# fims9000/SYNT_ISIC

Hardware: AMD Instinct MI355X
Metric: images/sec at 3x64x64 T=1000 (DDPM reverse-diffusion sampling) (higher is better)
Workload: dtype f32

## Files before the change

### synt_isic_amd/csrc/attention.hip

```cpp
#include <cstdlib>
#include <type_traits>

#include "common.h"

namespace sisic {

typedef float f32x16 __attribute__((ext_vector_type(16)));
typedef float f32x2 __attribute__((ext_vector_type(2)));
typedef short att_bf16x8 __attribute__((ext_vector_type(8)));
typedef unsigned att_u4 __attribute__((ext_vector_type(4)));
typedef unsigned att_u2 __attribute__((ext_vector_type(2)));

__device__ __forceinline__ void att_split2(float a, float b, unsigned& hi, unsigned& mid, unsigned& lo) {
    const unsigned ha = __float_as_uint(a) & 0xffff0000u, hb = __float_as_uint(b) & 0xffff0000u;
    const float ra = a - __uint_as_float(ha), rb = b - __uint_as_float(hb);
    const unsigned ma = __float_as_uint(ra) & 0xffff0000u, mb = __float_as_uint(rb) & 0xffff0000u;
    const float la = ra - __uint_as_float(ma), lb = rb - __uint_as_float(mb);
    hi = __builtin_amdgcn_perm(hb, ha, 0x07060302u);
    mid = __builtin_amdgcn_perm(mb, ma, 0x07060302u);
    lo = __builtin_amdgcn_perm(__float_as_uint(lb), __float_as_uint(la), 0x07060302u);
}

constexpr int ATT_D = 8;
constexpr int ATT_KB = 256;
constexpr int ATT_KT = ATT_KB / 32;
constexpr int ATT_WAVES = 4;

template <int QB>
__global__ void __launch_bounds__(64 * ATT_WAVES)
attention_kernel(const float* __restrict__ qkv, float* __restrict__ out, int C, int N, int heads, int q_blocks,
                 float scale) {
    __shared__ __attribute__((aligned(16))) unsigned Kh[2 * ATT_KB * 4];
    __shared__ __attribute__((aligned(16))) unsigned Kl[2 * ATT_KB * 2];
    __shared__ __attribute__((aligned(16))) float Vs[ATT_D * ATT_KB];

    int blk = blockIdx.x;
    const int qb = blk % q_blocks;
    blk /= q_blocks;
    const int head = blk % heads;
    const int b = blk / heads;

    const int tid = threadIdx.x, lane = tid & 63, wave = tid >> 6;
    const int half = lane >> 5, l31 = lane & 31;
    const int q0 = qb * (32 * QB * ATT_WAVES) + wave * (32 * QB);
    const bool wave_active = q0 < N;

    const float* Qp = qkv + ((size_t)b * 3 * C + (size_t)head * ATT_D) * N;
    const float* Kp = Qp + (size_t)C * N;
    const float* Vp = Kp + (size_t)C * N;

    att_u4 b_hm[QB], b_mh[QB], b_lh[QB];
#pragma unroll
    for (int j = 0; j < QB; ++j) {
        const int q = q0 + 32 * j + l31;
        float qv[4];
#pragma unroll
        for (int k = 0; k < 4; ++k) qv[k] = (q < N) ? Qp[(size_t)(4 * half + k) * N + q] * scale : 0.0f;
        unsigned h0, m0, l0, h1, m1, l1;
        att_split2(qv[0], qv[1], h0, m0, l0);
        att_split2(qv[2], qv[3], h1, m1, l1);
        b_hm[j] = att_u4{h0, h1, m0, m1};
        b_mh[j] = att_u4{m0, m1, h0, h1};
        b_lh[j] = att_u4{l0, l1, h0, h1};
    }

    float m_run[QB], l_part[QB];
    f32x2 o2[QB][ATT_D / 2];
#pragma unroll
    for (int j = 0; j < QB; ++j) {
        m_run[j] = -INFINITY; l_part[j] = 0.0f;
#pragma unroll
        for (int d = 0; d < ATT_D / 2; ++d) o2[j][d] = f32x2{0.0f, 0.0f};
    }

    auto tile = [&](const int kt, const int nk, auto masked) {
        constexpr bool MASKED = decltype(masked)::value;
        f32x16 S[QB];
        {
            const int key = half * ATT_KB + kt * 32 + l31;
            const att_u4 a_hm = *reinterpret_cast<const att_u4*>(&Kh[key * 4]);
            const att_u2 a_l = *reinterpret_cast<const att_u2*>(&Kl[key * 2]);
            const att_u4 a_hl = {a_hm.x, a_hm.y, a_l.x, a_l.y};
#pragma unroll
            for (int j = 0; j < QB; ++j) {
#pragma unroll
                for (int r = 0; r < 16; ++r) S[j][r] = 0.0f;
                S[j] = __builtin_amdgcn_mfma_f32_32x32x16_bf16(__builtin_bit_cast(att_bf16x8, a_hm), __builtin_bit_cast(att_bf16x8, b_hm[j]), S[j], 0, 0, 0);
                S[j] = __builtin_amdgcn_mfma_f32_32x32x16_bf16(__builtin_bit_cast(att_bf16x8, a_hm), __builtin_bit_cast(att_bf16x8, b_mh[j]), S[j], 0, 0, 0);
                S[j] = __builtin_amdgcn_mfma_f32_32x32x16_bf16(__builtin_bit_cast(att_bf16x8, a_hl), __builtin_bit_cast(att_bf16x8, b_lh[j]), S[j], 0, 0, 0);
            }
        }
        float m_new[QB];
#pragma unroll
        for (int j = 0; j < QB; ++j) {
            float tmax = -INFINITY;
#pragma unroll
            for (int r = 0; r < 16; ++r) {
                if (MASKED) {
                    const int key = kt * 32 + (r & 3) + 8 * (r >> 2) + 4 * half;
                    S[j][r] = (key < nk) ? S[j][r] : -INFINITY;
                }
                tmax = fmaxf(tmax, S[j][r]);
            }
            {
                const auto sw = __builtin_amdgcn_permlane32_swap(__float_as_uint(tmax), __float_as_uint(tmax), false, false);
                tmax = fmaxf(__uint_as_float(sw[0]), __uint_as_float(sw[1]));
            }
            m_new[j] = fmaxf(m_run[j], tmax);
            const float alpha = __builtin_amdgcn_exp2f(m_run[j] - m_new[j]);
            asm("s_nop 1\n\tv_mul_f32 %0, %1, %2" : "=v"(l_part[j]) : "v"(l_part[j]), "v"(alpha));
            const f32x2 a2 = f32x2{alpha, alpha};
#pragma unroll
            for (int d = 0; d < ATT_D / 2; ++d) asm("s_nop 1\n\tv_pk_mul_f32 %0, %1, %2" : "=v"(o2[j][d]) : "v"(o2[j][d]), "v"(a2));
            m_run[j] = m_new[j];
        }
#pragma unroll
        for (int rq = 0; rq < 4; ++rq) {
            float pv[QB][4];
#pragma unroll
            for (int j = 0; j < QB; ++j) {
                const f32x2 mm = f32x2{m_new[j], m_new[j]};
                const f32x2 d0 = f32x2{S[j][4 * rq], S[j][4 * rq + 1]} - mm, d1 = f32x2{S[j][4 * rq + 2], S[j][4 * rq + 3]} - mm;
                pv[j][0] = __builtin_amdgcn_exp2f(d0.x); pv[j][1] = __builtin_amdgcn_exp2f(d0.y);
                pv[j][2] = __builtin_amdgcn_exp2f(d1.x); pv[j][3] = __builtin_amdgcn_exp2f(d1.y);
                l_part[j] += (pv[j][0] + pv[j][1]) + (pv[j][2] + pv[j][3]);
            }
            const int koff = kt * 32 + 8 * rq + 4 * half;
#pragma unroll
            for (int i = 0; i < 4; ++i) {
                const float4 va = *reinterpret_cast<const float4*>(&Vs[(koff + i) * ATT_D]);
                const float4 vb = *reinterpret_cast<const float4*>(&Vs[(koff + i) * ATT_D + 4]);
#pragma unroll
                for (int j = 0; j < QB; ++j) {
                    const f32x2 p2 = f32x2{pv[j][i], pv[j][i]};
                    o2[j][0] += p2 * f32x2{va.x, va.y};
                    o2[j][1] += p2 * f32x2{va.z, va.w};
                    o2[j][2] += p2 * f32x2{vb.x, vb.y};
                    o2[j][3] += p2 * f32x2{vb.z, vb.w};
                }
            }
        }
    };

    for (int kb0 = 0; kb0 < N; kb0 += ATT_KB) {
        __syncthreads();
        for (int idx = tid; idx < 2 * ATT_KB; idx += 64 * ATT_WAVES) {
            const int g = idx / ATT_KB, k = idx % ATT_KB;
            const int key = kb0 + k;
            float kv[4];
#pragma unroll
            for (int d = 0; d < 4; ++d) kv[d] = key < N ? Kp[(size_t)(4 * g + d) * N + key] : 0.0f;
            unsigned h0, m0, l0, h1, m1, l1;
            att_split2(kv[0], kv[1], h0, m0, l0);
            att_split2(kv[2], kv[3], h1, m1, l1);
            *reinterpret_cast<att_u4*>(&Kh[idx * 4]) = att_u4{h0, h1, m0, m1};
            *reinterpret_cast<att_u2*>(&Kl[idx * 2]) = att_u2{l0, l1};
        }
        for (int k = tid; k < ATT_KB; k += 64 * ATT_WAVES) {
            const int key = kb0 + k;
            float v[ATT_D];
#pragma unroll
            for (int d = 0; d < ATT_D; ++d) v[d] = key < N ? Vp[(size_t)d * N + key] : 0.0f;
            *reinterpret_cast<float4*>(&Vs[k * ATT_D]) = make_float4(v[0], v[1], v[2], v[3]);
            *reinterpret_cast<float4*>(&Vs[k * ATT_D + 4]) = make_float4(v[4], v[5], v[6], v[7]);
        }
        __syncthreads();
        if (!wave_active) continue;
        const int nk = min(ATT_KB, N - kb0);
#pragma unroll 1
        for (int kt = 0; kt * 32 < nk; ++kt) {
            if (kt * 32 + 32 <= nk) tile(kt, nk, std::false_type{});
            else tile(kt, nk, std::true_type{});
        }
    }

    if (wave_active) {
#pragma unroll
        for (int j = 0; j < QB; ++j) {
            const int q = q0 + 32 * j + l31;
            float o[ATT_D];
#pragma unroll
            for (int d = 0; d < ATT_D / 2; ++d) { o[2 * d] = o2[j][d].x; o[2 * d + 1] = o2[j][d].y; }
            const float l_tot = l_part[j] + __shfl_xor(l_part[j], 32, 64);
            const float inv = 1.0f / l_tot;
            float res[ATT_D];
#pragma unroll
            for (int d = 0; d < ATT_D; ++d) res[d] = (o[d] + __shfl_xor(o[d], 32, 64)) * inv;
            if (q < N) {
                float* Op = out + ((size_t)b * C + (size_t)head * ATT_D) * N + q;
#pragma unroll
                for (int dd = 0; dd < 4; ++dd) {
                    const int hm = -half;
                    const float v = __int_as_float((__float_as_int(res[dd]) & ~hm) | (__float_as_int(res[4 + dd]) & hm));
                    Op[(size_t)(4 * half + dd) * N] = v;
                }
            }
        }
    }
}

int launch_attention(sisic_ctx* ctx, const float* qkv, float* out, int B, int C, int N, int head_dim, hipStream_t s) {
    SISIC_REQUIRE(qkv && out, "attention: null tensor");
    if (head_dim == 32 || head_dim == 64) return launch_attention_wide(ctx, qkv, out, B, C, N, head_dim, s);
    SISIC_REQUIRE(head_dim == ATT_D, "attention: head_dim %d unsupported (8, 32 and 64 have kernels)", head_dim);
    SISIC_REQUIRE(B > 0 && N > 0 && C > 0 && C % head_dim == 0, "attention: bad shape B=%d C=%d N=%d", B, C, N);
    const int heads = C / head_dim;
    static const int qb_env = [] { const char* e = std::getenv("SISIC_ATT_QB"); return e ? std::atoi(e) : 0; }();
    const int cus = ctx->num_cus > 0 ? ctx->num_cus : 256;
    const int qb = qb_env == 1 || qb_env == 2 ? qb_env : ((int64_t)B * heads * cdiv(N, 64 * ATT_WAVES) >= 4 * (int64_t)cus ? 2 : 1);
    const int q_blocks = cdiv(N, 32 * qb * ATT_WAVES);
    const int64_t grid = (int64_t)B * heads * q_blocks;
    SISIC_REQUIRE(grid < (int64_t(1) << 31), "attention: grid too large");
    ProfileScope prof(ctx, s, PK_ATTN, 16.0 * B * C * N, 4.0 * B * C * double(N) * N);
    const float scale = 1.4426950408889634f / sqrtf((float)head_dim);
    if (qb == 2)
        hipLaunchKernelGGL(attention_kernel<2>, dim3((unsigned)grid), dim3(64 * ATT_WAVES), 0, s, qkv, out, C, N, heads, q_blocks, scale);
    else
        hipLaunchKernelGGL(attention_kernel<1>, dim3((unsigned)grid), dim3(64 * ATT_WAVES), 0, s, qkv, out, C, N, heads, q_blocks, scale);
    SISIC_HIP(hipGetLastError());
    return SISIC_OK;
}

}
```

### synt_isic_amd/csrc/conv_pointwise_bf3.hip

```cpp
#include <cstdlib>
#include <type_traits>

#include "conv_plan.h"
#include "gn_finalize.h"

namespace sisic {

typedef float pwb_f32x16 __attribute__((ext_vector_type(16)));
typedef short pwb_bf16x8 __attribute__((ext_vector_type(8)));
typedef unsigned pwb_u4 __attribute__((ext_vector_type(4)));
typedef unsigned pwb_u2 __attribute__((ext_vector_type(2)));
typedef float pwb_f2 __attribute__((ext_vector_type(2)));
typedef float pwb_f4 __attribute__((ext_vector_type(4)));

struct PwbParams {
    const float* in0;
    const float* in1;
    int c0, c1, B, HW;
    const float* wb;
    int n_co64;
    const float* bias;
    int Cout;
    const float* gn_scale;
    const float* gn_shift;
// ... 246 lines not shown
            if (p.bias) add[r] += p.bias[col];
            if (p.chan_bias) add[r] += p.chan_bias[(size_t)b * p.chan_bias_stride + col];
            res[r] = pwb_f2{0.0f, 0.0f};
            if (p.residual) {
                if constexpr (NB == 2) res[r] = __builtin_bit_cast(pwb_f2, __builtin_amdgcn_raw_buffer_load_b64(rsr, o_voff, 4u * (unsigned)(cs * HW), 0));
                else res[r].x = __builtin_bit_cast(float, __builtin_amdgcn_raw_buffer_load_b32(rsr, o_voff, 4u * (unsigned)(cs * HW), 0));
            }
        }
#pragma unroll
        for (int r = 0; r < 16; ++r) {
            const int cs = co0 + 32 * x + 8 * (r >> 2) + (r & 3);
            float vv[2] = {0.0f, 0.0f};
#pragma unroll
            for (int nb = 0; nb < NB; ++nb) {
                vv[nb] = acc[x][nb][r] + add[r] + (nb ? res[r].y : res[r].x);
                if (p.relu) vv[nb] = fmaxf(vv[nb], 0.0f);
            }
            if constexpr (NB == 2) __builtin_amdgcn_raw_buffer_store_b64(pwb_u2{__float_as_uint(vv[0]), __float_as_uint(vv[1])}, rso, o_voff, 4u * (unsigned)(cs * HW), 0);
            else __builtin_amdgcn_raw_buffer_store_b32(__float_as_uint(vv[0]), rso, o_voff, 4u * (unsigned)(cs * HW), 0);
            if (p.stats) {
                const int co = cs + 4 * half;
                if constexpr (NB == 1) {
                    const float s1 = pwb_half_wave_sum(vv[0]);
                    const float d = vv[0] - s1 * (1.0f / 32.0f);
                    float dd;
                    asm volatile("v_mul_f32 %0, %1, %1" : "=v"(dd) : "v"(d));
                    const float q = pwb_half_wave_sum(dd);
                    if (l31 == 0)
                        reinterpret_cast<float4*>(p.stats)[((size_t)b * p.Cout + co) * slots + px_t] = make_float4(32.0f, s1, q, 0.0f);
                } else {
                    const float s1 = pwb_row16_sum(vv[0] + vv[1]);
                    const float mean = s1 * (1.0f / 32.0f);
                    const float d0 = vv[0] - mean, d1 = vv[1] - mean;
                    float q0, q1;
                    asm volatile("v_mul_f32 %0, %2, %2\n\tv_mul_f32 %1, %3, %3" : "=&v"(q0), "=&v"(q1) : "v"(d0), "v"(d1));
                    const float q = pwb_row16_sum(q0 + q1);
                    if ((l31 & 15) == 0)
                        reinterpret_cast<float4*>(p.stats)[((size_t)b * p.Cout + co) * slots + 2 * px_t + (l31 >> 4)] = make_float4(32.0f, s1, q, 0.0f);
                }
            }
        }
    }
}

#ifndef PWBK_VAR
#define PWBK_VAR 0
#endif
template <int PRO>
__global__ void __launch_bounds__(64 * PWB_WAVES, 4) conv_pwbk_kernel(const PwbParams p) {
    extern __shared__ __attribute__((aligned(16))) float smem[];
    int L = blockIdx.x;
    if constexpr (PRO == 0) {
        if (L < p.n_rider_wg) {
            gn_finalize_job(p.rider, L * GNF_WAVES + (int)(threadIdx.x >> 6), threadIdx.x & 63);
            return;
        }
        L -= p.n_rider_wg;
    }
    int item;
    {
        const int nwg = p.nwg;
        const int xcd = L & 7, slot = L >> 3, q = nwg >> 3, r = nwg & 7;
        item = (xcd < r ? xcd * (q + 1) : r * (q + 1) + (xcd - r) * q) + slot;
    }
    const int tid = threadIdx.x, lane = tid & 63;
    const int wave_u = __builtin_amdgcn_readfirstlane(tid >> 6);
    const int half = lane >> 5, l31 = lane & 31;
    int co_i = item % p.n_co_items;
    const int t = item / p.n_co_items;
    int px_t = t % p.n_px, b = t / p.n_px;
    asm volatile("" : "+s"(co_i), "+s"(px_t), "+s"(b));
    constexpr int CB = 2;
    const int px0 = 32 * px_t, co0 = 64 * co_i;
    const int Cin = p.c0 + p.c1, HW = p.HW;
    const int nl = p.nchunks / PWB_WAVES, cb = wave_u * nl;

    const __amdgpu_buffer_rsrc_t rs0 = __builtin_amdgcn_make_buffer_rsrc(const_cast<float*>(p.in0 + (size_t)b * p.c0 * HW), 0, -1, 0x00020000);
    const __amdgpu_buffer_rsrc_t rs1 = __builtin_amdgcn_make_buffer_rsrc(
        const_cast<float*>(p.in1 ? p.in1 + (size_t)b * p.c1 * HW : p.in0), 0, -1, 0x00020000);
    const __amdgpu_buffer_rsrc_t rsw = __builtin_amdgcn_make_buffer_rsrc(const_cast<float*>(p.wb), 0, -1, 0x00020000);
    const unsigned x_voff = 4u * (unsigned)((4 * half) * HW + px0 + l31);
    const unsigned a_lane16 = 16u * (unsigned)lane, a_lane8 = 8u * (unsigned)lane;

    float* const P_lds = smem;
    float* const gnL = smem + PWB_WAVES * 32 * 64 + wave_u * (2 * 8 * nl);
    if constexpr (PRO != 0) {
        for (int i = lane; i < 8 * nl; i += 64) {
            gnL[2 * i] = p.gn_scale[(size_t)b * Cin + 8 * cb + i];
            gnL[2 * i + 1] = p.gn_shift[(size_t)b * Cin + 8 * cb + i];
        }
        asm volatile("s_waitcnt lgkmcnt(0)" ::: "memory");
        __builtin_amdgcn_wave_barrier();
    }

    pwb_f32x16 acc[CB];
#pragma unroll
    for (int x = 0; x < CB; ++x)
#pragma unroll
        for (int r = 0; r < 16; ++r) acc[x][r] = 0.0f;
    struct XRegs { float x[4]; };
    auto load_x = [&](int c, XRegs& r) {
        const int cc0 = 8 * c;
        if (cc0 < p.c0) {
            const unsigned soff = 4u * (unsigned)(cc0 * HW);
#pragma unroll
            for (int k = 0; k < 4; ++k) r.x[k] = __builtin_bit_cast(float, __builtin_amdgcn_raw_buffer_load_b32(rs0, x_voff, soff + 4u * (unsigned)(k * HW), 0));
        } else {
            const unsigned soff = 4u * (unsigned)((cc0 - p.c0) * HW);
#pragma unroll
            for (int k = 0; k < 4; ++k) r.x[k] = __builtin_bit_cast(float, __builtin_amdgcn_raw_buffer_load_b32(rs1, x_voff, soff + 4u * (unsigned)(k * HW), 0));
        }
    };
    auto load_f = [&](int c, pwb_u4 (&fa)[CB], pwb_u2 (&fl)[CB]) {
        const unsigned s0 = 3072u * (unsigned)(c * p.n_co64 + co_i);
#pragma unroll
        for (int x = 0; x < CB; ++x) {
            fa[x] = __builtin_amdgcn_raw_buffer_load_b128(rsw, a_lane16, s0 + 1024u * (unsigned)x, 0);
#if (PWBK_VAR & 1) != 0
            fl[x] = pwb_u2{fa[x].z, fa[x].w};
#else
            fl[x] = __builtin_amdgcn_raw_buffer_load_b64(rsw, a_lane8, s0 + 2048u + 512u * (unsigned)x, 0);
#endif
#if (PWBK_VAR & 2) != 0
            fa[x] = pwb_u4{a_lane16 + (unsigned)c, a_lane8, s0, a_lane16 ^ s0};
            fl[x] = pwb_u2{fa[x].z, fa[x].w};
#endif
        }
    };
    struct Tup { pwb_u4 hm, mh, lh; };
    auto make = [&](int cl, const XRegs& r) {
        pwb_f4 g01 = {1.0f, 0.0f, 1.0f, 0.0f}, g23 = g01;
        if constexpr (PRO != 0) {
            const float* gp = gnL + 2 * (8 * cl + 4 * half);
            g01 = *reinterpret_cast<const pwb_f4*>(gp);
            g23 = *reinterpret_cast<const pwb_f4*>(gp + 4);
        }
        float v[4];
#pragma unroll
        for (int k = 0; k < 4; ++k) {
            float e = r.x[k];
            if constexpr (PRO != 0) {
                const float sc = k == 0 ? g01.x : (k == 1 ? g01.z : (k == 2 ? g23.x : g23.z));
                const float sh = k == 0 ? g01.y : (k == 1 ? g01.w : (k == 2 ? g23.y : g23.w));
                e = e * sc + sh;
                if constexpr (PRO == 2) e = pwb_silu(e);
            }
            v[k] = e;
        }
        unsigned hi[2], mid[2], lo[2];
#pragma unroll
        for (int q = 0; q < 2; ++q) {
            const float v0 = v[2 * q], v1 = v[2 * q + 1];
            const unsigned h0 = __float_as_uint(v0) & 0xffff0000u, h1 = __float_as_uint(v1) & 0xffff0000u;
            const float r0 = v0 - __uint_as_float(h0), r1 = v1 - __uint_as_float(h1);
            const unsigned m0 = __float_as_uint(r0) & 0xffff0000u, m1 = __float_as_uint(r1) & 0xffff0000u;
            const float l0 = r0 - __uint_as_float(m0), l1 = r1 - __uint_as_float(m1);
            hi[q] = __builtin_amdgcn_perm(h1, h0, 0x07060302u);
            mid[q] = __builtin_amdgcn_perm(m1, m0, 0x07060302u);
            lo[q] = __builtin_amdgcn_perm(__float_as_uint(l1), __float_as_uint(l0), 0x07060302u);
        }
        return Tup{pwb_u4{hi[0], hi[1], mid[0], mid[1]}, pwb_u4{mid[0], mid[1], hi[0], hi[1]}, pwb_u4{lo[0], lo[1], hi[0], hi[1]}};
    };
    auto mm = [&](const Tup& t, const pwb_u4 (&fa)[CB], const pwb_u2 (&fl)[CB]) {
#pragma unroll
        for (int x = 0; x < CB; ++x) {
            const pwb_u4 a_hl = {fa[x].x, fa[x].y, fl[x].x, fl[x].y};
            acc[x] = __builtin_amdgcn_mfma_f32_32x32x16_bf16(__builtin_bit_cast(pwb_bf16x8, fa[x]), __builtin_bit_cast(pwb_bf16x8, t.hm), acc[x], 0, 0, 0);
            acc[x] = __builtin_amdgcn_mfma_f32_32x32x16_bf16(__builtin_bit_cast(pwb_bf16x8, fa[x]), __builtin_bit_cast(pwb_bf16x8, t.mh), acc[x], 0, 0, 0);
            acc[x] = __builtin_amdgcn_mfma_f32_32x32x16_bf16(__builtin_bit_cast(pwb_bf16x8, a_hl), __builtin_bit_cast(pwb_bf16x8, t.lh), acc[x], 0, 0, 0);
        }
    };
    constexpr int XD = 4;
    XRegs xr[XD];
    pwb_u4 ua[CB], ub[CB];
    pwb_u2 ul[CB], um[CB];
#pragma unroll
    for (int i = 0; i < XD; ++i)
        if (i < nl) load_x(cb + i, xr[i]);
    load_f(cb, ua, ul);
    if (nl > 1) load_f(cb + 1, ub, um);
    for (int c = 0; c < nl; c += XD) {
#pragma unroll
        for (int i = 0; i < XD; ++i) {
            if (c + i < nl) {
                const Tup t = make(c + i, xr[i]);
                if (c + i + XD < nl) load_x(cb + c + i + XD, xr[i]);
                if ((i & 1) == 0) {
                    mm(t, ua, ul);
                    if (c + i + 2 < nl) load_f(cb + c + i + 2, ua, ul);
                } else {
                    mm(t, ub, um);
                    if (c + i + 2 < nl) load_f(cb + c + i + 2, ub, um);
                }
            }
        }
    }

#pragma unroll
    for (int x = 0; x < CB; ++x)
#pragma unroll
        for (int r = 0; r < 16; ++r) P_lds[((wave_u * 2 + x) * 16 + r) * 64 + lane] = acc[x][r];
    __syncthreads();
    const int x = wave_u >> 1, rb = 8 * (wave_u & 1);
    const __amdgpu_buffer_rsrc_t rso = __builtin_amdgcn_make_buffer_rsrc(p.out + (size_t)b * p.Cout * HW, 0, -1, 0x00020000);
    const __amdgpu_buffer_rsrc_t rsr = __builtin_amdgcn_make_buffer_rsrc(
        const_cast<float*>(p.residual ? p.residual + (size_t)b * p.Cout * HW : p.out), 0, -1, 0x00020000);
    const unsigned o_voff = 4u * (unsigned)((4 * half) * HW + px0 + l31);
    const int slots = HW / 32;
    float add[8], res[8];
#pragma unroll
    for (int rr = 0; rr < 8; ++rr) {
        const int r = rb + rr;
        const int cs = co0 + 32 * x + 8 * (r >> 2) + (r & 3);
        const int col = cs + 4 * half;
        add[rr] = 0.0f;
        if (p.bias) add[rr] += p.bias[col];
        if (p.chan_bias) add[rr] += p.chan_bias[(size_t)b * p.chan_bias_stride + col];
        res[rr] = 0.0f;
        if (p.residual) res[rr] = __builtin_bit_cast(float, __builtin_amdgcn_raw_buffer_load_b32(rsr, o_voff, 4u * (unsigned)(cs * HW), 0));
    }
#pragma unroll
    for (int rr = 0; rr < 8; ++rr) {
        const int r = rb + rr;
        const int cs = co0 + 32 * x + 8 * (r >> 2) + (r & 3);
        float part[PWB_WAVES];
#pragma unroll
        for (int k = 0; k < PWB_WAVES; ++k) part[k] = P_lds[((k * 2 + x) * 16 + r) * 64 + lane];
        float v = ((part[0] + part[1]) + part[2]) + part[3];
        v = v + add[rr] + res[rr];
        if (p.relu) v = fmaxf(v, 0.0f);
        __builtin_amdgcn_raw_buffer_store_b32(__float_as_uint(v), rso, o_voff, 4u * (unsigned)(cs * HW), 0);
        if (p.stats) {
            const int co = cs + 4 * half;
            const float s1 = pwb_half_wave_sum(v);
            const float d = v - s1 * (1.0f / 32.0f);
            float dd;
            asm volatile("v_mul_f32 %0, %1, %1" : "=v"(dd) : "v"(d));
            const float q = pwb_half_wave_sum(dd);
            if (l31 == 0)
                reinterpret_cast<float4*>(p.stats)[((size_t)b * p.Cout + co) * slots + px_t] = make_float4(32.0f, s1, q, 0.0f);
        }
    }
}

__device__ __forceinline__ void pwbs_load_chunk(const __amdgpu_buffer_rsrc_t rs0, const __amdgpu_buffer_rsrc_t rs1, const int c0, const int HW,
                                                const int c, const unsigned x_voff, pwb_f2 (&xr)[4]) {
    const int cc0 = 8 * c;
    if (cc0 < c0) {
        const unsigned soff = 4u * (unsigned)(cc0 * HW);
#pragma unroll
        for (int k = 0; k < 4; ++k) xr[k] = __builtin_bit_cast(pwb_f2, __builtin_amdgcn_raw_buffer_load_b64(rs0, x_voff, soff + 4u * (unsigned)(k * HW), 0));
    } else {
        const unsigned soff = 4u * (unsigned)((cc0 - c0) * HW);
#pragma unroll
        for (int k = 0; k < 4; ++k) xr[k] = __builtin_bit_cast(pwb_f2, __builtin_amdgcn_raw_buffer_load_b64(rs1, x_voff, soff + 4u * (unsigned)(k * HW), 0));
    }
}
template <int PRO>
__device__ __forceinline__ void pwbs_split_store(const pwb_f2 (&xr)[4], const float* gp, unsigned* const S_hm, unsigned* const S_lo, const int slot,
                                                 const int lane) {
    pwb_f4 g01 = {1.0f, 0.0f, 1.0f, 0.0f}, g23 = g01;
    if constexpr (PRO != 0) {
        g01 = *reinterpret_cast<const pwb_f4*>(gp);
        g23 = *reinterpret_cast<const pwb_f4*>(gp + 4);
    }
#pragma unroll
    for (int nb = 0; nb < 2; ++nb) {
        float v[4];
#pragma unroll
        for (int k = 0; k < 4; ++k) {
            float e = nb ? xr[k].y : xr[k].x;
            if constexpr (PRO != 0) {
                const float sc = k == 0 ? g01.x : (k == 1 ? g01.z : (k == 2 ? g23.x : g23.z));
                const float sh = k == 0 ? g01.y : (k == 1 ? g01.w : (k == 2 ? g23.y : g23.w));
                e = e * sc + sh;
                if constexpr (PRO == 2) e = pwb_silu(e);
            }
            v[k] = e;
        }
        unsigned hi[2], mid[2], lo[2];
#pragma unroll
        for (int q = 0; q < 2; ++q) {
            const float v0 = v[2 * q], v1 = v[2 * q + 1];
            const unsigned h0 = __float_as_uint(v0) & 0xffff0000u, h1 = __float_as_uint(v1) & 0xffff0000u;
            const float r0 = v0 - __uint_as_float(h0), r1 = v1 - __uint_as_float(h1);
            const unsigned m0 = __float_as_uint(r0) & 0xffff0000u, m1 = __float_as_uint(r1) & 0xffff0000u;
            const float l0 = r0 - __uint_as_float(m0), l1 = r1 - __uint_as_float(m1);
            hi[q] = __builtin_amdgcn_perm(h1, h0, 0x07060302u);
            mid[q] = __builtin_amdgcn_perm(m1, m0, 0x07060302u);
            lo[q] = __builtin_amdgcn_perm(__float_as_uint(l1), __float_as_uint(l0), 0x07060302u);
        }
        *reinterpret_cast<pwb_u4*>(S_hm + ((size_t)(slot * 2 + nb) * 64 + lane) * 4) = pwb_u4{hi[0], hi[1], mid[0], mid[1]};
        *reinterpret_cast<pwb_u2*>(S_lo + ((size_t)(slot * 2 + nb) * 64 + lane) * 2) = pwb_u2{lo[0], lo[1]};
    }
}
__device__ __forceinline__ void pwbs_read_b(const unsigned* const S_hm, const unsigned* const S_lo, const int slot, const int nb, const int lane,
                                            pwb_u4& hm, pwb_u4& mh, pwb_u4& lh) {
    hm = *reinterpret_cast<const pwb_u4*>(S_hm + ((size_t)(slot * 2 + nb) * 64 + lane) * 4);
    const pwb_u2 lo = *reinterpret_cast<const pwb_u2*>(S_lo + ((size_t)(slot * 2 + nb) * 64 + lane) * 2);
    mh = pwb_u4{hm.z, hm.w, hm.x, hm.y};
    lh = pwb_u4{lo.x, lo.y, hm.x, hm.y};
}

template <int PRO>
__global__ void __launch_bounds__(64 * PWBS_MAX_WAVES) conv_pwbs_kernel(const PwbParams p) {
    extern __shared__ __attribute__((aligned(16))) float smem[];
    int wg;
    {
        const int L = blockIdx.x, nwg = p.nwg;
        const int xcd = L & 7, slot = L >> 3, q = nwg >> 3, r = nwg & 7;
        wg = (xcd < r ? xcd * (q + 1) : r * (q + 1) + (xcd - r) * q) + slot;
    }
    const int tid = threadIdx.x, lane = tid & 63;
    const int wave_u = __builtin_amdgcn_readfirstlane(tid >> 6);
    const int nwaves = p.n_co_items;
    const int half = lane >> 5, l31 = lane & 31;
    int px_t = wg % p.n_px, b = wg / p.n_px;
    asm volatile("" : "+s"(px_t), "+s"(b));
    constexpr int CB = 2, NB = 2;
    const int co_i = wave_u;
    const int px0 = 64 * px_t, co0 = 64 * co_i;
    const int Cin = p.c0 + p.c1, HW = p.HW, n = p.nchunks;

    const __amdgpu_buffer_rsrc_t rs0 = __builtin_amdgcn_make_buffer_rsrc(const_cast<float*>(p.in0 + (size_t)b * p.c0 * HW), 0, -1, 0x00020000);
    const __amdgpu_buffer_rsrc_t rs1 = __builtin_amdgcn_make_buffer_rsrc(
        const_cast<float*>(p.in1 ? p.in1 + (size_t)b * p.c1 * HW : p.in0), 0, -1, 0x00020000);
    const __amdgpu_buffer_rsrc_t rsw = __builtin_amdgcn_make_buffer_rsrc(const_cast<float*>(p.wb), 0, -1, 0x00020000);
    const unsigned x_voff = 4u * (unsigned)((4 * half) * HW + px0 + NB * l31);
    const unsigned a_lane16 = 16u * (unsigned)lane, a_lane8 = 8u * (unsigned)lane;

    unsigned* const S_hm = reinterpret_cast<unsigned*>(smem);
    unsigned* const S_lo = S_hm + (size_t)n * NB * 64 * 4;
    float* const gnL = reinterpret_cast<float*>(S_lo + (size_t)n * NB * 64 * 2);
    if constexpr (PRO != 0) {
        for (int i = tid; i < Cin; i += 64 * nwaves) {
            gnL[2 * i] = p.gn_scale[(size_t)b * Cin + i];
            gnL[2 * i + 1] = p.gn_shift[(size_t)b * Cin + i];
        }
        __syncthreads();
    }
    for (int c = wave_u; c < n; c += nwaves) {
        pwb_f2 xr[4];
        pwbs_load_chunk(rs0, rs1, p.c0, HW, c, x_voff, xr);
        pwbs_split_store<PRO>(xr, gnL + 2 * (8 * c + 4 * half), S_hm, S_lo, c, lane);
    }
    __syncthreads();

    pwb_f32x16 acc[CB][NB];
#pragma unroll
    for (int x = 0; x < CB; ++x)
#pragma unroll
        for (int nb = 0; nb < NB; ++nb)
#pragma unroll
            for (int r = 0; r < 16; ++r) acc[x][nb][r] = 0.0f;
    pwb_u4 ua[CB], ub[CB];
    pwb_u2 ul[CB], um[CB];
    auto load_f = [&](int c, pwb_u4 (&fa)[CB], pwb_u2 (&fl)[CB]) {
        const unsigned s0 = 3072u * (unsigned)(c * p.n_co64 + co_i);
#pragma unroll
        for (int x = 0; x < CB; ++x) {
            fa[x] = __builtin_amdgcn_raw_buffer_load_b128(rsw, a_lane16, s0 + 1024u * (unsigned)x, 0);
            fl[x] = __builtin_amdgcn_raw_buffer_load_b64(rsw, a_lane8, s0 + 2048u + 512u * (unsigned)x, 0);
        }
    };
    auto chunk = [&](int c, const pwb_u4 (&fa)[CB], const pwb_u2 (&fl)[CB]) {
#pragma unroll
        for (int nb = 0; nb < NB; ++nb) {
            pwb_u4 hm, mh, lh;
            pwbs_read_b(S_hm, S_lo, c, nb, lane, hm, mh, lh);
#pragma unroll
            for (int x = 0; x < CB; ++x) {
                const pwb_u4 a_hl = {fa[x].x, fa[x].y, fl[x].x, fl[x].y};
                acc[x][nb] = __builtin_amdgcn_mfma_f32_32x32x16_bf16(__builtin_bit_cast(pwb_bf16x8, fa[x]), __builtin_bit_cast(pwb_bf16x8, hm), acc[x][nb], 0, 0, 0);
                acc[x][nb] = __builtin_amdgcn_mfma_f32_32x32x16_bf16(__builtin_bit_cast(pwb_bf16x8, fa[x]), __builtin_bit_cast(pwb_bf16x8, mh), acc[x][nb], 0, 0, 0);
                acc[x][nb] = __builtin_amdgcn_mfma_f32_32x32x16_bf16(__builtin_bit_cast(pwb_bf16x8, a_hl), __builtin_bit_cast(pwb_bf16x8, lh), acc[x][nb], 0, 0, 0);
            }
        }
    };
    load_f(0, ua, ul);
    if (n > 1) load_f(1, ub, um);
    {
        int c = 0;
        for (; c + 1 < n; c += 2) {
            chunk(c, ua, ul);
            if (c + 2 < n) load_f(c + 2, ua, ul);
            chunk(c + 1, ub, um);
            if (c + 3 < n) load_f(c + 3, ub, um);
        }
        if (c < n) chunk(c, ua, ul);
    }

    const __amdgpu_buffer_rsrc_t rso = __builtin_amdgcn_make_buffer_rsrc(p.out + (size_t)b * p.Cout * HW, 0, -1, 0x00020000);
    const __amdgpu_buffer_rsrc_t rsr = __builtin_amdgcn_make_buffer_rsrc(
        const_cast<float*>(p.residual ? p.residual + (size_t)b * p.Cout * HW : p.out), 0, -1, 0x00020000);
    const unsigned o_voff = 4u * (unsigned)((4 * half) * HW + px0 + NB * l31);
    const int slots = HW / 32;
#pragma unroll
    for (int x = 0; x < CB; ++x) {
        float add[16];
        pwb_f2 res[16];
#pragma unroll
        for (int r = 0; r < 16; ++r) {
            const int cs = co0 + 32 * x + 8 * (r >> 2) + (r & 3);
            const int col = cs + 4 * half;
            add[r] = 0.0f;
            if (p.bias) add[r] += p.bias[col];
            if (p.chan_bias) add[r] += p.chan_bias[(size_t)b * p.chan_bias_stride + col];
            res[r] = pwb_f2{0.0f, 0.0f};
            if (p.residual) res[r] = __builtin_bit_cast(pwb_f2, __builtin_amdgcn_raw_buffer_load_b64(rsr, o_voff, 4u * (unsigned)(cs * HW), 0));
        }
#pragma unroll
        for (int r = 0; r < 16; ++r) {
            const int cs = co0 + 32 * x + 8 * (r >> 2) + (r & 3);
            float vv[2];
#pragma unroll
            for (int nb = 0; nb < NB; ++nb) {
                vv[nb] = acc[x][nb][r] + add[r] + (nb ? res[r].y : res[r].x);
                if (p.relu) vv[nb] = fmaxf(vv[nb], 0.0f);
            }
            __builtin_amdgcn_raw_buffer_store_b64(pwb_u2{__float_as_uint(vv[0]), __float_as_uint(vv[1])}, rso, o_voff, 4u * (unsigned)(cs * HW), 0);
            if (p.stats) {
                const int co = cs + 4 * half;
                const float s1 = pwb_row16_sum(vv[0] + vv[1]);
                const float mean = s1 * (1.0f / 32.0f);
                const float d0 = vv[0] - mean, d1 = vv[1] - mean;
                float q0, q1;
                asm volatile("v_mul_f32 %0, %2, %2\n\tv_mul_f32 %1, %3, %3" : "=&v"(q0), "=&v"(q1) : "v"(d0), "v"(d1));
                const float q = pwb_row16_sum(q0 + q1);
                if ((l31 & 15) == 0)
                    reinterpret_cast<float4*>(p.stats)[((size_t)b * p.Cout + co) * slots + 2 * px_t + (l31 >> 4)] = make_float4(32.0f, s1, q, 0.0f);
            }
        }
    }
}

#ifndef PWBSK_VAR
#define PWBSK_VAR 0
#endif
__global__ void __launch_bounds__(64 * PWBSK_MAX_WAVES) conv_pwbsk_kernel(const PwbParams p) {
    extern __shared__ __attribute__((aligned(16))) float smem[];
    const int tid = threadIdx.x, lane = tid & 63;
    const int wave_u = __builtin_amdgcn_readfirstlane(tid >> 6);
    const int nwaves = PWB_WAVES * p.n_co_items;
    int L = blockIdx.x;
    if (L < p.n_rider_wg) {
        gn_finalize_job(p.rider, L * nwaves + wave_u, lane);
        return;
    }
    L -= p.n_rider_wg;
    int wg;
    {
        const int nwg = p.nwg;
        const int xcd = L & 7, slot = L >> 3, q = nwg >> 3, r = nwg & 7;
        wg = (xcd < r ? xcd * (q + 1) : r * (q + 1) + (xcd - r) * q) + slot;
    }
    const int half = lane >> 5, l31 = lane & 31;
    int px_t = wg % p.n_px, b = wg / p.n_px;
    asm volatile("" : "+s"(px_t), "+s"(b));
    constexpr int CB = 2, NB = 2;
    const int co_i = wave_u / PWB_WAVES, kq = wave_u % PWB_WAVES;
    const int px0 = 64 * px_t, co0 = 64 * co_i;
    const int HW = p.HW;
    const int nl = p.nchunks / PWB_WAVES, cb = kq * nl;
    const int cap = nl < PWBSK_CAP ? nl : PWBSK_CAP;

    const __amdgpu_buffer_rsrc_t rs0 = __builtin_amdgcn_make_buffer_rsrc(const_cast<float*>(p.in0 + (size_t)b * p.c0 * HW), 0, -1, 0x00020000);
    const __amdgpu_buffer_rsrc_t rs1 = __builtin_amdgcn_make_buffer_rsrc(
        const_cast<float*>(p.in1 ? p.in1 + (size_t)b * p.c1 * HW : p.in0), 0, -1, 0x00020000);
    const __amdgpu_buffer_rsrc_t rsw = __builtin_amdgcn_make_buffer_rsrc(const_cast<float*>(p.wb), 0, -1, 0x00020000);
    const unsigned x_voff = 4u * (unsigned)((4 * half) * HW + px0 + NB * l31);
    const unsigned a_lane16 = 16u * (unsigned)lane, a_lane8 = 8u * (unsigned)lane;

    unsigned* const S_hm = reinterpret_cast<unsigned*>(smem);
    unsigned* const S_lo = S_hm + (size_t)(PWB_WAVES * cap) * NB * 64 * 4;
    float* const P_lds = smem;

    pwb_f32x16 acc[CB][NB];
#pragma unroll
    for (int x = 0; x < CB; ++x)
#pragma unroll
        for (int nb = 0; nb < NB; ++nb)
#pragma unroll
            for (int r = 0; r < 16; ++r) acc[x][nb][r] = 0.0f;
    pwb_u4 ua[CB], ub[CB];
    pwb_u2 ul[CB], um[CB];
    auto load_f = [&](int c, pwb_u4 (&fa)[CB], pwb_u2 (&fl)[CB]) {
        const unsigned s0 = 3072u * (unsigned)(c * p.n_co64 + co_i);
#pragma unroll
        for (int x = 0; x < CB; ++x) {
#if (PWBSK_VAR & 8) != 0
            fa[x] = pwb_u4{a_lane16 + (unsigned)c, a_lane8, s0, a_lane16 ^ s0};
            fl[x] = pwb_u2{fa[x].z, fa[x].w};
#else
            fa[x] = __builtin_amdgcn_raw_buffer_load_b128(rsw, a_lane16, s0 + 1024u * (unsigned)x, 0);
            fl[x] = __builtin_amdgcn_raw_buffer_load_b64(rsw, a_lane8, s0 + 2048u + 512u * (unsigned)x, 0);
#endif
        }
    };
    auto chunk = [&](int slot, const pwb_u4 (&fa)[CB], const pwb_u2 (&fl)[CB]) {
#pragma unroll
        for (int nb = 0; nb < NB; ++nb) {
            pwb_u4 hm, mh, lh;
            pwbs_read_b(S_hm, S_lo, slot, nb, lane, hm, mh, lh);
#pragma unroll
            for (int x = 0; x < CB; ++x) {
                const pwb_u4 a_hl = {fa[x].x, fa[x].y, fl[x].x, fl[x].y};
                acc[x][nb] = __builtin_amdgcn_mfma_f32_32x32x16_bf16(__builtin_bit_cast(pwb_bf16x8, fa[x]), __builtin_bit_cast(pwb_bf16x8, hm), acc[x][nb], 0, 0, 0);
                acc[x][nb] = __builtin_amdgcn_mfma_f32_32x32x16_bf16(__builtin_bit_cast(pwb_bf16x8, fa[x]), __builtin_bit_cast(pwb_bf16x8, mh), acc[x][nb], 0, 0, 0);
                acc[x][nb] = __builtin_amdgcn_mfma_f32_32x32x16_bf16(__builtin_bit_cast(pwb_bf16x8, a_hl), __builtin_bit_cast(pwb_bf16x8, lh), acc[x][nb], 0, 0, 0);
            }
        }
    };
    load_f(cb, ua, ul);
    load_f(cb + 1, ub, um);
    for (int p0 = 0; p0 < nl; p0 += cap) {
        const int len = nl - p0 < cap ? nl - p0 : cap, nslots = PWB_WAVES * len;
        if (p0 != 0) __syncthreads();
#if (PWBSK_VAR & 1) == 0
        for (int t = wave_u; t < nslots; t += 2 * nwaves) {
            const int t1 = t + nwaves;
            pwb_f2 xa[4], xb[4];
            pwbs_load_chunk(rs0, rs1, p.c0, HW, (t / len) * nl + p0 + t % len, x_voff, xa);
            if (t1 < nslots) pwbs_load_chunk(rs0, rs1, p.c0, HW, (t1 / len) * nl + p0 + t1 % len, x_voff, xb);
            pwbs_split_store<0>(xa, nullptr, S_hm, S_lo, (t / len) * cap + t % len, lane);
            if (t1 < nslots) pwbs_split_store<0>(xb, nullptr, S_hm, S_lo, (t1 / len) * cap + t1 % len, lane);
        }
#endif
        __syncthreads();
#if (PWBSK_VAR & 2) == 0
        for (int j = 0; j < len; j += 2) {
            chunk(kq * cap + j, ua, ul);
            if (p0 + j + 2 < nl) load_f(cb + p0 + j + 2, ua, ul);
            chunk(kq * cap + j + 1, ub, um);
            if (p0 + j + 3 < nl) load_f(cb + p0 + j + 3, ub, um);
        }
#else
        acc[0][0][0] += __uint_as_float(ua[0].x ^ ub[1].y ^ ul[0].x ^ um[1].y) + __uint_as_float(S_hm[lane + 64 * kq]);
#endif
    }

    const __amdgpu_buffer_rsrc_t rso = __builtin_amdgcn_make_buffer_rsrc(p.out + (size_t)b * p.Cout * HW, 0, -1, 0x00020000);
    const __amdgpu_buffer_rsrc_t rsr = __builtin_amdgcn_make_buffer_rsrc(
        const_cast<float*>(p.residual ? p.residual + (size_t)b * p.Cout * HW : p.out), 0, -1, 0x00020000);
    const unsigned o_voff = 4u * (unsigned)((4 * half) * HW + px0 + NB * l31);
    const int slots = HW / 32;
#pragma unroll
    for (int x = 0; x < CB; ++x) {
#if (PWBSK_VAR & 4) == 0
        __syncthreads();
#pragma unroll
        for (int nb = 0; nb < NB; ++nb)
#pragma unroll
            for (int r = 0; r < 16; ++r) P_lds[((wave_u * NB + nb) * 16 + r) * 64 + lane] = acc[x][nb][r];
        __syncthreads();
#endif
        float add[4];
        pwb_f2 res[4];
#pragma unroll
        for (int rr = 0; rr < 4; ++rr) {
            const int cs = co0 + 32 * x + 8 * kq + rr;
            const int col = cs + 4 * half;
            add[rr] = 0.0f;
            if (p.bias) add[rr] += p.bias[col];
            if (p.chan_bias) add[rr] += p.chan_bias[(size_t)b * p.chan_bias_stride + col];
            res[rr] = pwb_f2{0.0f, 0.0f};
            if (p.residual) res[rr] = __builtin_bit_cast(pwb_f2, __builtin_amdgcn_raw_buffer_load_b64(rsr, o_voff, 4u * (unsigned)(cs * HW), 0));
        }
#pragma unroll
        for (int rr = 0; rr < 4; ++rr) {
            const int r = 4 * kq + rr;
            const int cs = co0 + 32 * x + 8 * kq + rr;
            float vv[NB];
#pragma unroll
            for (int nb = 0; nb < NB; ++nb) {
                float part[PWB_WAVES];
#if (PWBSK_VAR & 4) == 0
#pragma unroll
                for (int k = 0; k < PWB_WAVES; ++k) part[k] = P_lds[(((co_i * PWB_WAVES + k) * NB + nb) * 16 + r) * 64 + lane];
#else
#pragma unroll
                for (int k = 0; k < PWB_WAVES; ++k) part[k] = acc[x][nb][4 * k + rr];
#endif
                float v = ((part[0] + part[1]) + part[2]) + part[3];
                v = v + add[rr] + (nb ? res[rr].y : res[rr].x);
                vv[nb] = v;
            }
            __builtin_amdgcn_raw_buffer_store_b64(pwb_u2{__float_as_uint(vv[0]), __float_as_uint(vv[1])}, rso, o_voff, 4u * (unsigned)(cs * HW), 0);
            if (p.stats) {
                const int co = cs + 4 * half;
                const float s1 = pwb_row16_sum(vv[0] + vv[1]);
                const float mean = s1 * (1.0f / 32.0f);
                const float d0 = vv[0] - mean, d1 = vv[1] - mean;
                float q0, q1;
                asm volatile("v_mul_f32 %0, %2, %2\n\tv_mul_f32 %1, %3, %3" : "=&v"(q0), "=&v"(q1) : "v"(d0), "v"(d1));
                const float q = pwb_row16_sum(q0 + q1);
                if ((l31 & 15) == 0)
                    reinterpret_cast<float4*>(p.stats)[((size_t)b * p.Cout + co) * slots + 2 * px_t + (l31 >> 4)] = make_float4(32.0f, s1, q, 0.0f);
            }
        }
    }
}

static int launch_pwbsk(sisic_ctx* ctx, PwbParams& p, int Cin, hipStream_t s, const GnFinJob* rider) {
    p.n_co_items = p.Cout / 64;
    p.n_px = p.HW / 64;
    const int nwaves = PWB_WAVES * p.n_co_items;
    const int64_t nwg = (int64_t)p.B * p.n_px;
    p.n_rider_wg = rider ? cdiv(rider->n_jobs, nwaves) : 0;
    SISIC_REQUIRE(nwg > 0 && nwg + p.n_rider_wg < (int64_t(1) << 31), "conv2d(pointwise bf16x3, staged K-split): grid too large");
    p.nwg = (int)nwg;
    p.nitems = p.nwg * p.n_co_items;
    const size_t lds = pwbsk_lds_bytes(Cin, p.Cout);
    static std::atomic<uint64_t> opt{0};
    auto kern = conv_pwbsk_kernel;
    SISIC_TRY(ensure_dynamic_lds(ctx, reinterpret_cast<const void*>(kern), (int)PWBSK_MAX_LDS, opt));
    hipLaunchKernelGGL(kern, dim3(p.n_rider_wg + p.nwg), dim3(64 * nwaves), lds, s, p);
    SISIC_HIP(hipGetLastError());
    return SISIC_OK;
}

template <int PRO>
static int launch_pwbk(sisic_ctx* ctx, PwbParams& p, int Cin, hipStream_t s) {
    p.n_co_items = p.Cout / 64;
    p.n_px = p.HW / 32;
    const int64_t nitems = (int64_t)p.B * p.n_px * p.n_co_items;
    SISIC_REQUIRE(nitems > 0 && nitems < (int64_t(1) << 31), "conv2d(pointwise bf16x3, K-split): grid too large");
    p.nitems = (int)nitems;
    p.nwg = p.nitems;
    SISIC_REQUIRE((int64_t)p.nwg + p.n_rider_wg < (int64_t(1) << 31), "conv2d(pointwise bf16x3, K-split): grid too large");
    const size_t lds = sizeof(float) * (size_t)(PWB_WAVES * 32 * 64 + (PRO ? 2 * Cin : 0));
    static std::atomic<uint64_t> opt{0};
    auto kern = conv_pwbk_kernel<PRO>;
    SISIC_TRY(ensure_dynamic_lds(ctx, reinterpret_cast<const void*>(kern), (int)lds, opt));
    hipLaunchKernelGGL(kern, dim3(p.n_rider_wg + p.nwg), dim3(64 * PWB_WAVES), lds, s, p);
    SISIC_HIP(hipGetLastError());
    return SISIC_OK;
}

template <int PRO>
static int launch_pwbs(sisic_ctx* ctx, PwbParams& p, int Cin, hipStream_t s) {
    p.n_co_items = p.Cout / 64;
    p.n_px = p.HW / 64;
    const int64_t nwg = (int64_t)p.B * p.n_px;
    SISIC_REQUIRE(nwg > 0 && nwg < (int64_t(1) << 31), "conv2d(pointwise bf16x3, staged): grid too large");
    p.nwg = (int)nwg;
    p.nitems = p.nwg * p.n_co_items;
    const size_t lds = pwbs_lds_bytes(Cin);
    static std::atomic<uint64_t> opt{0};
    auto kern = conv_pwbs_kernel<PRO>;
    SISIC_TRY(ensure_dynamic_lds(ctx, reinterpret_cast<const void*>(kern), (int)lds, opt));
    hipLaunchKernelGGL(kern, dim3(p.nwg), dim3(64 * p.n_co_items), lds, s, p);
    SISIC_HIP(hipGetLastError());
    return SISIC_OK;
}

bool conv_pointwise_bf3_applicable(const sisic_conv_args& a) {
    if (a.ksize != 1 || a.stride != 1 || a.upsample) return false;
    const int HW = a.Hin * a.Win, Cin = a.c0 + a.c1;
    if (HW % 64 != 0 || Cin % 8 != 0 || (a.c1 != 0 && a.c0 % 8 != 0) || a.Cout % 64 != 0) return false;
    if (((reinterpret_cast<uintptr_t>(a.in0) | reinterpret_cast<uintptr_t>(a.in1) | reinterpret_cast<uintptr_t>(a.out) |
          reinterpret_cast<uintptr_t>(a.residual)) & 7) != 0) return false;
    if (4.0 * std::max(std::max(a.c0, a.c1), a.Cout) * HW >= 4294967296.0 || 6.0 * conv_cin_pad(Cin, 1) * conv_cout_pad(a.Cout) >= 4294967296.0) return false;
    if (a.gn_scale && Cin > 1024) return false;
    return true;
}

template <int PRO, int NB>
static int launch_pwb(sisic_ctx* ctx, PwbParams& p, int Cin, hipStream_t s) {
    p.n_co_items = p.Cout / 64;
    p.n_px = p.HW / (32 * NB);
    const int64_t nitems = (int64_t)p.B * p.n_px * p.n_co_items;
    SISIC_REQUIRE(nitems > 0 && nitems < (int64_t(1) << 31), "conv2d(pointwise bf16x3): grid too large");
    p.nitems = (int)nitems;
    p.nwg = (int)((nitems + PWB_WAVES - 1) / PWB_WAVES);
    SISIC_REQUIRE((int64_t)p.nwg + p.n_rider_wg < (int64_t(1) << 31), "conv2d(pointwise bf16x3): grid too large");
    const size_t lds = PRO ? sizeof(float) * (size_t)(PWB_WAVES * 2 * Cin) : 0;
    static std::atomic<uint64_t> opt{0};
    auto kern = conv_pwb_kernel<PRO, NB>;
    SISIC_TRY(ensure_dynamic_lds(ctx, reinterpret_cast<const void*>(kern), (int)lds, opt));
    hipLaunchKernelGGL(kern, dim3(p.n_rider_wg + p.nwg), dim3(64 * PWB_WAVES), lds, s, p);
    SISIC_HIP(hipGetLastError());
    return SISIC_OK;
}

int launch_conv_pointwise_bf3(sisic_ctx* ctx, const sisic_conv_args& a, const ConvPlan& plan, hipStream_t s, const GnFinJob* rider) {
    PwbParams p{};
    const int Cin = a.c0 + a.c1;
    p.in0 = a.in0; p.in1 = a.in1; p.c0 = a.c0; p.c1 = a.c1; p.B = a.B; p.HW = a.Hin * a.Win;
    p.wb = a.w_packed + 2 * (size_t)conv_cin_pad(Cin, 1) * conv_cout_pad(a.Cout);
    p.n_co64 = conv_cout_pad(a.Cout) / 64;
    p.bias = a.bias; p.Cout = a.Cout;
    p.gn_scale = a.gn_scale; p.gn_shift = a.gn_shift;
    p.chan_bias = a.chan_bias; p.chan_bias_stride = a.chan_bias_stride; p.residual = a.residual; p.relu = a.relu;
// ... 21 lines not shown
```

Before: 12.66.

## Pack multiple attention heads per block when sequence is short

After: 12.69, median of 6. No clear change (+0.3%).

```diff
diff --git a/synt_isic_amd/csrc/attention.hip b/synt_isic_amd/csrc/attention.hip
--- a/synt_isic_amd/csrc/attention.hip
+++ b/synt_isic_amd/csrc/attention.hip
@@ -26,10 +26,12 @@
 constexpr int ATT_KT = ATT_KB / 32;
 constexpr int ATT_WAVES = 4;
 
-template <int QB>
+template <int QB, int HPW>
 __global__ void __launch_bounds__(64 * ATT_WAVES)
 attention_kernel(const float* __restrict__ qkv, float* __restrict__ out, int C, int N, int heads, int q_blocks,
                  float scale) {
+    constexpr int KBP = ATT_KB / HPW;
+    constexpr int WPH = ATT_WAVES / HPW;
     __shared__ __attribute__((aligned(16))) unsigned Kh[2 * ATT_KB * 4];
     __shared__ __attribute__((aligned(16))) unsigned Kl[2 * ATT_KB * 2];
     __shared__ __attribute__((aligned(16))) float Vs[ATT_D * ATT_KB];
@@ -37,17 +39,23 @@
     int blk = blockIdx.x;
     const int qb = blk % q_blocks;
     blk /= q_blocks;
-    const int head = blk % heads;
-    const int b = blk / heads;
+    const int hgroups = (heads + HPW - 1) / HPW;
+    const int head0 = (blk % hgroups) * HPW;
+    const int b = blk / hgroups;
 
     const int tid = threadIdx.x, lane = tid & 63, wave = tid >> 6;
     const int half = lane >> 5, l31 = lane & 31;
-    const int q0 = qb * (32 * QB * ATT_WAVES) + wave * (32 * QB);
-    const bool wave_active = q0 < N;
-
+    const int hl = wave / WPH, head = head0 + hl;
+    const int q0 = qb * (32 * QB * WPH) + (wave % WPH) * (32 * QB);
+    const bool head_ok = HPW == 1 || head < heads;
+    const bool wave_active = head_ok && q0 < N;
+
+    const float* Kp = qkv + ((size_t)b * 3 * C + (size_t)C + (size_t)head0 * ATT_D) * N;
+    const float* Vp = Kp + (size_t)C * N;
     const float* Qp = qkv + ((size_t)b * 3 * C + (size_t)head * ATT_D) * N;
-    const float* Kp = Qp + (size_t)C * N;
-    const float* Vp = Kp + (size_t)C * N;
+    const unsigned* const Khp = Kh + hl * (2 * KBP * 4);
+    const unsigned* const Klp = Kl + hl * (2 * KBP * 2);
+    const float* const Vsp = Vs + hl * (KBP * ATT_D);
 
     att_u4 b_hm[QB], b_mh[QB], b_lh[QB];
 #pragma unroll
@@ -55,7 +63,7 @@
         const int q = q0 + 32 * j + l31;
         float qv[4];
 #pragma unroll
-        for (int k = 0; k < 4; ++k) qv[k] = (q < N) ? Qp[(size_t)(4 * half + k) * N + q] * scale : 0.0f;
+        for (int k = 0; k < 4; ++k) qv[k] = (head_ok && q < N) ? Qp[(size_t)(4 * half + k) * N + q] * scale : 0.0f;
         unsigned h0, m0, l0, h1, m1, l1;
         att_split2(qv[0], qv[1], h0, m0, l0);
         att_split2(qv[2], qv[3], h1, m1, l1);
@@ -77,9 +85,9 @@
         constexpr bool MASKED = decltype(masked)::value;
         f32x16 S[QB];
         {
-            const int key = half * ATT_KB + kt * 32 + l31;
-            const att_u4 a_hm = *reinterpret_cast<const att_u4*>(&Kh[key * 4]);
-            const att_u2 a_l = *reinterpret_cast<const att_u2*>(&Kl[key * 2]);
+            const int key = half * KBP + kt * 32 + l31;
+            const att_u4 a_hm = *reinterpret_cast<const att_u4*>(&Khp[key * 4]);
+            const att_u2 a_l = *reinterpret_cast<const att_u2*>(&Klp[key * 2]);
             const att_u4 a_hl = {a_hm.x, a_hm.y, a_l.x, a_l.y};
 #pragma unroll
             for (int j = 0; j < QB; ++j) {
@@ -128,8 +136,8 @@
             const int koff = kt * 32 + 8 * rq + 4 * half;
 #pragma unroll
             for (int i = 0; i < 4; ++i) {
-                const float4 va = *reinterpret_cast<const float4*>(&Vs[(koff + i) * ATT_D]);
-                const float4 vb = *reinterpret_cast<const float4*>(&Vs[(koff + i) * ATT_D + 4]);
+                const float4 va = *reinterpret_cast<const float4*>(&Vsp[(koff + i) * ATT_D]);
+                const float4 vb = *reinterpret_cast<const float4*>(&Vsp[(koff + i) * ATT_D + 4]);
 #pragma unroll
                 for (int j = 0; j < QB; ++j) {
                     const f32x2 p2 = f32x2{pv[j][i], pv[j][i]};
@@ -142,14 +150,15 @@
         }
     };
 
-    for (int kb0 = 0; kb0 < N; kb0 += ATT_KB) {
+    for (int kb0 = 0; kb0 < N; kb0 += KBP) {
         __syncthreads();
         for (int idx = tid; idx < 2 * ATT_KB; idx += 64 * ATT_WAVES) {
-            const int g = idx / ATT_KB, k = idx % ATT_KB;
+            const int h = idx / (2 * KBP), g = (idx / KBP) % 2, k = idx % KBP;
             const int key = kb0 + k;
+            const bool ok = key < N && (HPW == 1 || head0 + h < heads);
             float kv[4];
 #pragma unroll
-            for (int d = 0; d < 4; ++d) kv[d] = key < N ? Kp[(size_t)(4 * g + d) * N + key] : 0.0f;
+            for (int d = 0; d < 4; ++d) kv[d] = ok ? Kp[(size_t)(ATT_D * h + 4 * g + d) * N + key] : 0.0f;
             unsigned h0, m0, l0, h1, m1, l1;
             att_split2(kv[0], kv[1], h0, m0, l0);
             att_split2(kv[2], kv[3], h1, m1, l1);
@@ -157,16 +166,18 @@
             *reinterpret_cast<att_u2*>(&Kl[idx * 2]) = att_u2{l0, l1};
         }
         for (int k = tid; k < ATT_KB; k += 64 * ATT_WAVES) {
-            const int key = kb0 + k;
+            const int h = k / KBP;
+            const int key = kb0 + k % KBP;
+            const bool ok = key < N && (HPW == 1 || head0 + h < heads);
             float v[ATT_D];
 #pragma unroll
-            for (int d = 0; d < ATT_D; ++d) v[d] = key < N ? Vp[(size_t)d * N + key] : 0.0f;
+            for (int d = 0; d < ATT_D; ++d) v[d] = ok ? Vp[(size_t)(ATT_D * h + d) * N + key] : 0.0f;
             *reinterpret_cast<float4*>(&Vs[k * ATT_D]) = make_float4(v[0], v[1], v[2], v[3]);
             *reinterpret_cast<float4*>(&Vs[k * ATT_D + 4]) = make_float4(v[4], v[5], v[6], v[7]);
         }
         __syncthreads();
         if (!wave_active) continue;
-        const int nk = min(ATT_KB, N - kb0);
+        const int nk = min(KBP, N - kb0);
 #pragma unroll 1
         for (int kt = 0; kt * 32 < nk; ++kt) {
             if (kt * 32 + 32 <= nk) tile(kt, nk, std::false_type{});
@@ -206,17 +217,19 @@
     SISIC_REQUIRE(B > 0 && N > 0 && C > 0 && C % head_dim == 0, "attention: bad shape B=%d C=%d N=%d", B, C, N);
     const int heads = C / head_dim;
     static const int qb_env = [] { const char* e = std::getenv("SISIC_ATT_QB"); return e ? std::atoi(e) : 0; }();
+    static const bool share_env = [] { const char* e = std::getenv("SISIC_ATT_SHARE"); return !(e && e[0] == '0'); }();
     const int cus = ctx->num_cus > 0 ? ctx->num_cus : 256;
     const int qb = qb_env == 1 || qb_env == 2 ? qb_env : ((int64_t)B * heads * cdiv(N, 64 * ATT_WAVES) >= 4 * (int64_t)cus ? 2 : 1);
-    const int q_blocks = cdiv(N, 32 * qb * ATT_WAVES);
-    const int64_t grid = (int64_t)B * heads * q_blocks;
+    const int wph = cdiv(N, 32 * qb);
+    const int hpw = !share_env || wph > 2 ? 1 : ATT_WAVES / wph;
+    const int q_blocks = cdiv(N, 32 * qb * (ATT_WAVES / hpw));
+    const int64_t grid = (int64_t)B * cdiv(heads, hpw) * q_blocks;
     SISIC_REQUIRE(grid < (int64_t(1) << 31), "attention: grid too large");
     ProfileScope prof(ctx, s, PK_ATTN, 16.0 * B * C * N, 4.0 * B * C * double(N) * N);
     const float scale = 1.4426950408889634f / sqrtf((float)head_dim);
-    if (qb == 2)
-        hipLaunchKernelGGL(attention_kernel<2>, dim3((unsigned)grid), dim3(64 * ATT_WAVES), 0, s, qkv, out, C, N, heads, q_blocks, scale);
-    else
-        hipLaunchKernelGGL(attention_kernel<1>, dim3((unsigned)grid), dim3(64 * ATT_WAVES), 0, s, qkv, out, C, N, heads, q_blocks, scale);
+    auto kern = qb == 2 ? (hpw == 4 ? attention_kernel<2, 4> : hpw == 2 ? attention_kernel<2, 2> : attention_kernel<2, 1>)
+                        : (hpw == 4 ? attention_kernel<1, 4> : hpw == 2 ? attention_kernel<1, 2> : attention_kernel<1, 1>);
+    hipLaunchKernelGGL(kern, dim3((unsigned)grid), dim3(64 * ATT_WAVES), 0, s, qkv, out, C, N, heads, q_blocks, scale);
     SISIC_HIP(hipGetLastError());
     return SISIC_OK;
 }
diff --git a/synt_isic_amd/csrc/conv_pointwise_bf3.hip b/synt_isic_amd/csrc/conv_pointwise_bf3.hip
--- a/synt_isic_amd/csrc/conv_pointwise_bf3.hip
+++ b/synt_isic_amd/csrc/conv_pointwise_bf3.hip
@@ -572,6 +572,9 @@
     lh = pwb_u4{lo.x, lo.y, hm.x, hm.y};
 }
 
+#ifndef PWBS_VAR
+#define PWBS_VAR 0
+#endif
 template <int PRO>
 __global__ void __launch_bounds__(64 * PWBS_MAX_WAVES) conv_pwbs_kernel(const PwbParams p) {
     extern __shared__ __attribute__((aligned(16))) float smem[];
@@ -602,6 +605,7 @@
     unsigned* const S_hm = reinterpret_cast<unsigned*>(smem);
     unsigned* const S_lo = S_hm + (size_t)n * NB * 64 * 4;
     float* const gnL = reinterpret_cast<float*>(S_lo + (size_t)n * NB * 64 * 2);
+#if (PWBS_VAR & 1) == 0
     if constexpr (PRO != 0) {
         for (int i = tid; i < Cin; i += 64 * nwaves) {
             gnL[2 * i] = p.gn_scale[(size_t)b * Cin + i];
@@ -614,6 +618,7 @@
         pwbs_load_chunk(rs0, rs1, p.c0, HW, c, x_voff, xr);
         pwbs_split_store<PRO>(xr, gnL + 2 * (8 * c + 4 * half), S_hm, S_lo, c, lane);
     }
+#endif
     __syncthreads();
 
     pwb_f32x16 acc[CB][NB];
@@ -629,8 +634,13 @@
         const unsigned s0 = 3072u * (unsigned)(c * p.n_co64 + co_i);
 #pragma unroll
         for (int x = 0; x < CB; ++x) {
+#if (PWBS_VAR & 4) != 0
+            fa[x] = pwb_u4{a_lane16 + (unsigned)c, a_lane8, s0, a_lane16 ^ s0};
+            fl[x] = pwb_u2{fa[x].z, fa[x].w};
+#else
             fa[x] = __builtin_amdgcn_raw_buffer_load_b128(rsw, a_lane16, s0 + 1024u * (unsigned)x, 0);
             fl[x] = __builtin_amdgcn_raw_buffer_load_b64(rsw, a_lane8, s0 + 2048u + 512u * (unsigned)x, 0);
+#endif
         }
     };
     auto chunk = [&](int c, const pwb_u4 (&fa)[CB], const pwb_u2 (&fl)[CB]) {
@@ -649,6 +659,7 @@
     };
     load_f(0, ua, ul);
     if (n > 1) load_f(1, ub, um);
+#if (PWBS_VAR & 2) == 0
     {
         int c = 0;
         for (; c + 1 < n; c += 2) {
@@ -659,6 +670,9 @@
         }
         if (c < n) chunk(c, ua, ul);
     }
+#else
+    acc[0][0][0] += __uint_as_float(ua[0].x ^ ub[1].y ^ ul[0].x ^ um[1].y) + __uint_as_float(S_hm[lane + 64 * wave_u]);
+#endif
 
     const __amdgpu_buffer_rsrc_t rso = __builtin_amdgcn_make_buffer_rsrc(p.out + (size_t)b * p.Cout * HW, 0, -1, 0x00020000);
     const __amdgpu_buffer_rsrc_t rsr = __builtin_amdgcn_make_buffer_rsrc(
```
